# mitschabaude/msm-zprize

Measured on AMD Instinct MI355X. Metric: Mpoint-adds/s (ms per MSM in ms_per_step), higher is better.
Workload: dtype u32 limbs (28-bit lazy Montgomery, i64 accumulate)

## Files before the change

### msm_zprize_amd/_native.py

```python
import ctypes as C
import os

HERE = os.path.dirname(os.path.abspath(__file__))
LIB_PATH = os.environ.get("MSMZ_LIB") or os.path.join(HERE, "libmsmz.so")

MSMZ_N_STAGES = 8
STAGE_NAMES = ["digits", "scan", "scatter", "plan", "accumulate", "reduce", "final", "total"]


class MsmzOpts(C.Structure):
    _fields_ = [("c", C.c_int32), ("glv", C.c_int32), ("safe", C.c_int32), ("buckets", C.c_int32),
                ("timing", C.c_int32), ("reserved", C.c_int32 * 3)]


class MsmzLog(C.Structure):
    _fields_ = [("stage_ms", C.c_float * MSMZ_N_STAGES), ("c", C.c_int32), ("K", C.c_int32), ("rounds", C.c_int32),
                ("glv", C.c_int32), ("n_entries", C.c_uint64), ("n_pairs", C.c_uint64), ("max_bucket", C.c_uint32),
                ("scatter_launches", C.c_uint32), ("scatter_kernel_ms", C.c_float), ("batch_add_ms", C.c_float * 32)]


MSMZ_SRC_DEVICE, MSMZ_SRC_MONTGOMERY, MSMZ_SRC_DEFAULT_STREAM = 1, 2, 4
MSMZ_SRC_COMPRESSED, MSMZ_SRC_SIGN_PARITY = 8, 16
MSMZ_ERR_POINT = 7

# ... 24 lines not shown


class MsmzScalarTerm(C.Structure):
    _fields_ = [("handle", C.c_uint64), ("first", C.c_uint64), ("coeff_handle", C.c_uint64), ("coeff_first", C.c_uint64),
                ("coeff", C.c_char_p)]


MSMZ_REC_REVERSE, MSMZ_REC_EXCLUSIVE = 1, 2


class MsmzScalarRec(C.Structure):
    _fields_ = [("a_handle", C.c_uint64), ("a_first", C.c_uint64), ("a", C.c_char_p), ("b_handle", C.c_uint64),
                ("b_first", C.c_uint64), ("init", C.c_char_p), ("flags", C.c_uint32)]


MSMZ_NTT_INVERSE, MSMZ_NTT_COSET = 1, 2


class MsmzNtt(C.Structure):
    _fields_ = [("handle", C.c_uint64), ("first", C.c_uint64), ("log_n", C.c_uint32), ("flags", C.c_uint32),
                ("n_in", C.c_uint64), ("count", C.c_uint32), ("root", C.c_char_p), ("shift", C.c_char_p)]


class MsmzSegment(C.Structure):
    _fields_ = [("first_p", C.c_uint64), ("first_s", C.c_uint64), ("n", C.c_uint64)]


class MsmzTestReduceArgs(C.Structure):
    _fields_ = [("mode", C.c_int32), ("c", C.c_int32), ("nsets", C.c_uint32), ("n_in", C.c_uint32),
                ("nc", C.c_uint32), ("tail_n", C.c_uint32), ("quad16_max", C.c_uint32), ("pairsum_x4_max", C.c_uint32),
                ("points_xy", C.c_char_p), ("points_inf", C.c_char_p), ("n_points", C.c_uint64),
                ("slots_xy", C.c_char_p), ("slots_inf", C.c_char_p), ("n_slots", C.c_uint64),
                ("scale", C.c_char_p), ("loc", C.c_void_p), ("cscan", C.c_void_p),
                ("out_xy", C.c_void_p), ("lines_xy", C.c_void_p)]


class MsmzTestPlanArgs(C.Structure):
    _fields_ = [("nb", C.c_uint32), ("chunk", C.c_uint32), ("nb_main", C.c_uint32), ("chunk_top", C.c_uint32),
                ("tail_skip", C.c_int32), ("reserved", C.c_uint32),
                ("off", C.c_void_p), ("refs", C.c_void_p),
                ("desc_cap", C.c_uint64), ("bfin_cap", C.c_uint64), ("chunk_pairs_cap", C.c_uint64),
                ("meta", C.c_void_p), ("desc", C.c_void_p), ("bfin", C.c_void_p), ("chunk_pairs", C.c_void_p)]


class MsmzTestSortArgs(C.Structure):
    _fields_ = [("scalars_le32", C.c_void_p), ("n", C.c_uint64), ("pts_n", C.c_uint64),
                ("nprob", C.c_uint32), ("factor", C.c_uint32), ("copy_stride", C.c_uint32),
                ("c", C.c_int32), ("glv", C.c_int32), ("force_fallback", C.c_int32), ("scalar_bits", C.c_int32),
                ("allow_fold", C.c_int32),
                ("geom_cap", C.c_uint64), ("off_cap", C.c_uint64), ("refs_cap", C.c_uint64), ("bins_cap", C.c_uint64),
                ("packed_cap", C.c_uint64),
                ("geom", C.c_void_p), ("meta", C.c_void_p), ("off", C.c_void_p), ("refs", C.c_void_p),
                ("bins", C.c_void_p), ("packed", C.c_void_p)]


TEST_SORT_GEOM = ["c", "K", "Keff", "L", "nb", "fb", "fbt", "ncb", "ncbt", "nbins", "sbins", "fbins", "fine_top", "spread",
                  "fold_shift", "fold_rows", "F", "mbits", "idx_bits", "cspec", "two_level", "tiles", "sbits", "endo_delta"]


EXPORTS = {
    "msmz_create": (C.c_int, [C.POINTER(C.c_void_p), C.c_int, C.POINTER(C.c_int), C.c_int]),
    "msmz_destroy": (None, [C.c_void_p]),
    "msmz_strerror": (C.c_char_p, [C.c_int]),
    "msmz_curve_fe_bytes": (C.c_int, [C.c_int]),
    "msmz_ctx_fe_bytes": (C.c_int, [C.c_void_p]),
    "msmz_ctx_n_devices": (C.c_int, [C.c_void_p]),
    "msmz_upload_points": (C.c_int, [C.c_void_p, C.c_char_p, C.c_char_p, C.c_uint64, C.POINTER(C.c_uint64)]),
# ... 21 lines not shown
                                    C.POINTER(MsmzOpts), C.c_char_p, C.POINTER(C.c_int), C.POINTER(MsmzLog)]),
    "msmz_precompute_points": (C.c_int, [C.c_void_p, C.c_uint64, C.c_uint64, C.POINTER(MsmzOpts), C.c_uint32,
                                         C.POINTER(C.c_uint64)]),
    "msmz_precomputed_info": (C.c_int, [C.c_void_p, C.c_uint64, C.POINTER(C.c_int32), C.POINTER(C.c_int32),
                                        C.POINTER(C.c_uint32), C.POINTER(C.c_uint32), C.POINTER(C.c_uint64)]),
    "msmz_precomputed_scalar_bits": (C.c_int, [C.c_void_p, C.c_uint64, C.POINTER(C.c_int32)]),
    "msmz_check_points": (C.c_int, [C.c_void_p, C.c_uint64, C.c_uint64, C.c_uint64, C.c_uint32,
                                    C.POINTER(MsmzCheckResult), C.c_char_p]),
    "msmz_points_mul": (C.c_int, [C.c_void_p, C.POINTER(MsmzMul), C.c_uint64, C.POINTER(C.c_uint64)]),
    "msmz_points_mul_opts": (C.c_int, [C.c_void_p, C.POINTER(MsmzMul), C.c_uint64, C.POINTER(MsmzMulOpts),
                                       C.POINTER(C.c_uint64)]),
    "msmz_scalars_combine": (C.c_int, [C.c_void_p, C.POINTER(MsmzScalarTerm), C.POINTER(MsmzScalarTerm), C.c_uint64,
                                       C.c_uint64, C.POINTER(C.c_uint64)]),
    "msmz_scalars_dot": (C.c_int, [C.c_void_p, C.c_uint64, C.c_uint64, C.c_uint64, C.c_uint64, C.c_uint64, C.c_char_p]),
    "msmz_scalars_powers": (C.c_int, [C.c_void_p, C.c_char_p, C.c_char_p, C.c_uint64, C.POINTER(C.c_uint64)]),
    "msmz_scalars_recurrence": (C.c_int, [C.c_void_p, C.POINTER(MsmzScalarRec), C.c_uint64, C.c_uint64,
                                          C.POINTER(C.c_uint64), C.c_char_p]),
    "msmz_scalars_inverse": (C.c_int, [C.c_void_p, C.c_uint64, C.c_uint64, C.c_uint64, C.c_uint64, C.POINTER(C.c_uint64),
                                       C.POINTER(C.c_uint64)]),
    "msmz_scalars_ntt": (C.c_int, [C.c_void_p, C.POINTER(MsmzNtt), C.c_uint64, C.POINTER(C.c_uint64)]),
    "msmz_scalars_root_of_unity": (C.c_int, [C.c_int, C.c_uint32, C.c_char_p]),
    "msmz_point_add": (C.c_int, [C.c_int, C.c_char_p, C.c_int, C.c_char_p, C.c_int, C.c_char_p, C.POINTER(C.c_int)]),
    "msmz_test_set_glv_bits": (C.c_int, [C.c_void_p, C.c_int]),
    "msmz_test_retries": (C.c_int, [C.c_void_p]),
    "msmz_test_set_limits": (C.c_int, [C.c_void_p, C.c_uint64, C.c_uint64]),
    "msmz_test_passes": (C.c_int, [C.c_void_p, C.POINTER(C.c_uint64), C.POINTER(C.c_uint64)]),
    "msmz_test_scalar_dot_geometry": (None, [C.POINTER(C.c_uint32), C.POINTER(C.c_uint32)]),
    "msmz_test_scalar_scan_geometry": (None, [C.POINTER(C.c_uint32), C.POINTER(C.c_uint32), C.POINTER(C.c_uint32)]),
    "msmz_test_ntt_plan": (C.c_int, [C.c_int, C.c_uint32, C.POINTER(C.c_uint32), C.POINTER(C.c_uint32)]),
    "msmz_test_ntt_geometry": (None, [C.POINTER(C.c_uint32)]),
    "msmz_test_field": (C.c_int, [C.c_void_p, C.c_int, C.c_char_p, C.c_char_p, C.c_uint64, C.c_char_p]),
    "msmz_test_field_limbs": (C.c_int, [C.c_void_p, C.c_int, C.c_void_p, C.c_void_p, C.c_uint64, C.c_void_p,
                                        C.c_char_p]),
    "msmz_test_glv": (C.c_int, [C.c_void_p, C.c_char_p, C.c_uint64, C.c_char_p, C.c_char_p, C.c_char_p]),
    "msmz_test_digits": (C.c_int, [C.c_void_p, C.c_char_p, C.c_uint64, C.c_int, C.c_int, C.c_int, C.c_void_p]),
    "msmz_test_sort": (C.c_int, [C.c_void_p, C.c_char_p, C.c_uint64, C.c_int, C.c_int, C.c_int, C.c_void_p, C.c_void_p,
                                 C.c_uint64, C.c_void_p, C.c_uint64]),
    "msmz_test_sort_ex": (C.c_int, [C.c_void_p, C.POINTER(MsmzTestSortArgs)]),
    "msmz_test_point_raw": (C.c_int, [C.c_void_p, C.c_int, C.c_char_p, C.c_char_p, C.c_char_p, C.c_uint64, C.c_int,
                                      C.c_char_p]),
    "msmz_test_point": (C.c_int, [C.c_void_p, C.c_int, C.c_char_p, C.c_char_p, C.c_char_p, C.c_char_p, C.c_uint64,
                                  C.c_char_p]),
    "msmz_test_batch_add": (C.c_int, [C.c_void_p, C.c_int, C.c_int, C.c_char_p, C.c_char_p, C.c_uint64, C.c_char_p,
                                      C.c_char_p, C.c_uint64, C.c_void_p, C.c_uint64, C.c_uint64, C.c_char_p,
                                      C.POINTER(C.c_uint32)]),
    "msmz_test_reduce": (C.c_int, [C.c_void_p, C.POINTER(MsmzTestReduceArgs)]),
    "msmz_test_plan": (C.c_int, [C.c_void_p, C.POINTER(MsmzTestPlanArgs)]),
}

_lib = None


class MsmzError(RuntimeError):
    def __init__(self, status, where):
        self.status = status
        msg = lib().msmz_strerror(status).decode() if _lib is not None else "?"
        super().__init__(f"{where}: msmz status {status} ({msg})")


def lib():
    global _lib
    if _lib is None:
        if not os.path.exists(LIB_PATH):
            raise RuntimeError(f"{LIB_PATH} is missing: run `python -m msm_zprize_amd.build` "
                               "(the MSM has no CPU fallback)")
        l = C.CDLL(LIB_PATH)
# ... 12 lines not shown
```

### msm_zprize_amd/csrc/instantiate.h

```cpp
#pragma once
#include "check_kernels.h"
#include "gen_kernels.h"
#include "import_kernels.h"
#include "kernels.h"
#include "mul_kernels.h"
#include "ntt_kernels.h"
#include "scalar_kernels.h"
#include "scan_kernels.h"
#include "test_kernels.h"

#if !defined(MSMZ_CURVE) || MSMZ_CURVE == 0
#define MSMZ_W0(X) X(Bls377Fp, Bls377Fr)
#else
#define MSMZ_W0(X)
#endif
#if !defined(MSMZ_CURVE) || MSMZ_CURVE == 1
#define MSMZ_W1(X) X(PallasFp, PallasFr)
#else
#define MSMZ_W1(X)
#endif
#if !defined(MSMZ_CURVE) || MSMZ_CURVE == 2
#define MSMZ_W2(X) X(Bls381Fp, Bls381Fr)
#else
#define MSMZ_W2(X)
#endif
#if !defined(MSMZ_CURVE) || MSMZ_CURVE == 3
#define MSMZ_T3(X) X(Ed377Fp, Ed377Fr)
#else
#define MSMZ_T3(X)
#endif
#define MSMZ_WEIERSTRASS_FIELDS(X) MSMZ_W0(X) MSMZ_W1(X) MSMZ_W2(X)
#define MSMZ_TE_FIELDS(X) MSMZ_T3(X)

#ifndef MSMZ_BATCH_T
#define MSMZ_BATCH_T 256
#endif
#ifndef MSMZ_BATCH_OCC
#define MSMZ_BATCH_OCC 4
#endif
#ifndef MSMZ_BATCH_BMAX
#define MSMZ_BATCH_BMAX 16
#endif

#define MSMZ_INST_BATCH(F, Fr, PFX)                                                                               \
  PFX template __global__ void k_batch_add<F, MSMZ_BATCH_T, true, MSMZ_BATCH_OCC, MSMZ_BATCH_BMAX>(              \
      uint32_t*, const uint32_t*, const uint2*, uint32_t, uint32_t, int, MsmMeta*);                              \
  PFX template __global__ void k_batch_add<F, MSMZ_BATCH_T, false, MSMZ_BATCH_OCC, MSMZ_BATCH_BMAX>(             \
      uint32_t*, const uint32_t*, const uint2*, uint32_t, uint32_t, int, MsmMeta*);

#define MSMZ_INST_POLICY(P, PFX)                                                                                 \
  PFX template __global__ void k_reduce_quad<P>(uint32_t*, uint32_t*, const uint32_t*, const uint32_t*, uint32_t, \
                                                uint32_t, uint32_t);                                             \
  PFX template __global__ void k_reduce_quad16<P>(uint32_t*, uint32_t*, const uint32_t*, const uint32_t*,        \
                                                  uint32_t, uint32_t, uint32_t);                                 \
  PFX template __global__ void k_reduce_tail<P>(uint32_t*, uint32_t*, uint32_t*, uint32_t*, uint32_t*, uint32_t, \
                                                uint32_t);                                                       \
  PFX template __global__ void k_pairsum<P>(uint32_t*, const uint32_t*, uint32_t);                               \
  PFX template __global__ void k_fill_neutral<P>(uint32_t*, uint32_t);                                           \
  PFX template __global__ void k_bucket_sums<P>(uint32_t*, const uint32_t*, const uint32_t*, uint32_t);          \
  PFX template __global__ void k_reduce2d_partial_acc<P>(uint32_t*, const uint32_t*, const uint32_t*, R2Geom, uint32_t); \
  PFX template __global__ void k_pairsum_x4<P>(uint32_t*, const uint32_t*, uint32_t);                            \
  PFX template __global__ void k_bucket_accumulate<P>(uint32_t*, const uint32_t*, const uint32_t*,               \
                                                      const uint32_t*, const uint32_t*, uint32_t, uint32_t, int);

#define MSMZ_INST_REDUCE(F, Fr, PFX)                                                                              \
  PFX template __global__ void k_reduce2d_partial<F>(uint32_t*, const uint32_t*, const uint32_t*, const uint4*,   \
                                                     R2Geom, uint32_t);                                          \
  PFX template __global__ void k_reduce_affine_finish<F>(uint32_t*, uint32_t*, const uint32_t*, const uint32_t*,  \
                                                         const uint2*, const uint4*, F2Geom);                     \
  MSMZ_INST_POLICY(WeierPolicy<F>, PFX)

#define MSMZ_INST_REDUCE_TE(F, Fr, PFX) MSMZ_INST_POLICY(TePolicy<F>, PFX)

#define MSMZ_INST_TEST(F, Fr, P, PFX)                                                                             \
  PFX template __global__ void k_test_field<F>(uint32_t*, const uint32_t*, const uint32_t*, uint32_t, int, uint32_t*); \
  PFX template __global__ void k_test_field_limbs<F>(int32_t*, uint32_t*, const int32_t*, const int32_t*, uint32_t,  \
                                                      int, uint32_t*);                                            \
  PFX template __global__ void k_test_glv<Fr>(uint32_t*, uint32_t*, uint8_t*, const uint32_t*, uint32_t);         \
  PFX template __global__ void k_test_digits<Fr, false>(uint32_t*, const uint32_t*, uint32_t, int, int);          \
  PFX template __global__ void k_test_point<P>(uint32_t*, const uint32_t*, const uint32_t*, const uint8_t*,   \
                                                   const uint8_t*, uint32_t, int);                                \
  PFX template __global__ void k_test_point_raw<P>(uint32_t*, const uint32_t*, const uint32_t*, const uint8_t*, \
                                                       uint32_t, int, int);                                       \
  PFX template __global__ void k_test_accs_in<P>(uint32_t*, const uint32_t*, const uint8_t*, const uint32_t*, \
                                                     uint32_t, uint32_t*);                                        \
  PFX template __global__ void k_test_accs_out<P>(uint32_t*, const uint32_t*, uint32_t);

#define MSMZ_INST_SORT(Fr, PFX, GLV, C, SEG)                                                                      \
  PFX template __global__ void k_hist<Fr, GLV, C, SEG>(uint32_t*, uint16_t*, uint32_t*, MsmMeta*, const uint32_t*, SortGeom, uint32_t, const SegDesc*); \
  PFX template __global__ void k_coarse<Fr, GLV, C, SEG>(uint32_t*, const uint32_t*, const uint32_t*, const uint16_t*, const uint32_t*, SortGeom, uint32_t, const SegDesc*);

#define MSMZ_INST_SCAN(Fr, AM, HB, PFX)                                                                           \
  PFX template __global__ void k_scalars_rec_tile<Fr, AM, HB>(uint32_t*, uint32_t*, const uint32_t*, const uint32_t*, FrConst, uint32_t, uint32_t, uint32_t*); \
  PFX template __global__ void k_scalars_rec_apply<Fr, AM, HB>(uint32_t*, const uint32_t*, const uint32_t*, FrConst, const uint32_t*, uint32_t, uint32_t);

#define MSMZ_INST_SCALAR(Fr, PFX)                                                                                 \
  PFX template __global__ void k_digits<Fr, false>(uint32_t*, uint32_t*, MsmMeta*, const uint32_t*, uint32_t, int, int, int, int); \
  MSMZ_SORT_INSTANCES(MSMZ_INST_SORT, Fr, PFX)                                                                    \
  PFX template __global__ void k_check_scalars<Fr>(uint32_t*, const uint32_t*, uint32_t);                         \
  PFX template __global__ void k_gen_scalars<Fr>(uint32_t*, uint32_t, uint64_t, GenMap);                          \
  PFX template __global__ void k_import_scalars<Fr>(uint32_t*, const uint8_t*, uint64_t, int, uint32_t, int, uint32_t*); \
  PFX template __global__ void k_scalars_combine<Fr>(uint32_t*, ScalarTerm, ScalarTerm, uint32_t, uint32_t*);     \
  PFX template __global__ void k_scalars_dot<Fr>(uint32_t*, const uint32_t*, const uint32_t*, uint32_t, uint32_t*); \
  PFX template __global__ void k_scalars_dot_fold<Fr>(uint32_t*, const uint32_t*, uint32_t, int);                 \
  PFX template __global__ void k_scalars_powers<Fr>(uint32_t*, FrConst, FrPowTable, uint32_t, GenMap);                \
  MSMZ_INST_SCAN(Fr, SREC_A_NONE, true, PFX)                                                                      \
  MSMZ_INST_SCAN(Fr, SREC_A_BROADCAST, false, PFX)                                                                \
  MSMZ_INST_SCAN(Fr, SREC_A_BROADCAST, true, PFX)                                                                 \
  MSMZ_INST_SCAN(Fr, SREC_A_RESIDENT, false, PFX)                                                                 \
  MSMZ_INST_SCAN(Fr, SREC_A_RESIDENT, true, PFX)                                                                  \
// ... 40 lines not shown
```

### msm_zprize_amd/csrc/kernels.h

```cpp
#pragma once
#include <hip/hip_runtime.h>
#include "constants_gen.h"
#include "plan.h"
#include "curve.h"
#include "scalar.h"

namespace msmz {

constexpr uint32_t REF_NEG = 0x80000000u;
constexpr uint32_t REF_IDX = 0x7fffffffu;

struct MsmMeta {
  uint32_t max_bucket;
  uint32_t n_entries;
  uint32_t error;
  uint32_t rounds;
  uint32_t round_pairs[32];
  uint32_t round_base[32];
};

typedef uint32_t u32x4 __attribute__((ext_vector_type(4)));

#ifndef MSMZ_POINT_PAD
#define MSMZ_POINT_PAD 1
#endif
template <class F>
struct PointFmt {
  static constexpr int STRIDE = (MSMZ_POINT_PAD && 2 * F::NW == 24) ? 32 : 2 * F::NW;
};

constexpr bool SLOT_NT = false;
template <class F, bool NT = false>
__device__ __forceinline__ void load_words(uint32_t* dst, const uint32_t* src, int cs = 1) {
  const u32x4* s4 = reinterpret_cast<const u32x4*>(src);
#pragma unroll
  for (int i = 0; i < (2 * F::NW) / 4; i++) {
    u32x4 v = NT ? __builtin_nontemporal_load(s4 + i * cs) : s4[i * cs];
// ... 367 lines not shown
template <class F>
__device__ __forceinline__ void load_operand_x(Fe<F>& x, uint32_t loc, const uint32_t* slots, const uint32_t* points) {
  if constexpr (SlotFmt<F>::PACKED) {
    int cs;
    uint32_t neg;
    const u32x4* s4 = reinterpret_cast<const u32x4*>(operand_address<F>(loc, slots, points, cs, neg));
    uint32_t w[F::NW];
#pragma unroll
    for (int i = 0; i < F::NW / 4; i++) {
      const u32x4 v = s4[i * cs];
      w[4 * i] = v.x;
      w[4 * i + 1] = v.y;
      w[4 * i + 2] = v.z;
      w[4 * i + 3] = v.w;
    }
    fe_unpack<F>(x, w);
  } else {
    if (loc & LOC_ORIG) {
      uint32_t w[F::NW];
      const u32x4* s4 = reinterpret_cast<const u32x4*>(points + (size_t)(loc & 0x3fffffffu) * PointFmt<F>::STRIDE);
#pragma unroll
      for (int i = 0; i < F::NW / 4; i++) {
        const u32x4 v = s4[i];
        w[4 * i] = v.x;
        w[4 * i + 1] = v.y;
        w[4 * i + 2] = v.z;
        w[4 * i + 3] = v.w;
      }
      fe_unpack<F>(x, w);
    } else {
      slot_load_fe<F>(x, slots + slot_offset<F>(loc));
    }
  }
}

template <int W, int N>
__device__ __forceinline__ int32_t limb_row_ripple(int32_t val, int j) {
  constexpr int32_t MASK = (1 << W) - 1;
  const bool low = j < N - 1;
#pragma unroll 1
  for (int pass = 0; pass < N - 1; pass++) {
    const int32_t c = low ? (val >> W) : 0;
    val = low ? (val & MASK) : val;
    val += __builtin_amdgcn_update_dpp(0, c, 0x111, 0xf, 0xf, true);
    if (__ballot(low && (uint32_t)val > (uint32_t)MASK) == 0) break;
  }
  return val;
}

template <class F>
__device__ __forceinline__ bool fe_inverse_wave(Fe<F>& r, const Fe<F>& x) {
  constexpr int N = F::N, W = F::W;
  constexpr uint32_t MASK = (1u << W) - 1u;
  static_assert(N <= 15, "one DPP row per vector");
  const int lane = (int)(threadIdx.x & 63u);
  const int row = lane >> 4, j = lane & 15;
  int32_t xl = 0, pl = 0, npl = 0;
  {
    Fe<F> xc;
    uint32_t w[F::NW];
    fe_to_canon_words<F>(w, x);
    fe_unpack<F>(xc, w);
#pragma unroll
    for (int k = 0; k < N; k++) {
      if (j == k) {
        xl = xc.l[k];
        pl = F::PL[k];
        npl = F::NPL[k];
      }
    }
  }
  int32_t val = row == 0 ? xl : row == 1 ? pl : (row == 2 && j == 0) ? 1 : 0;
  constexpr int ITERS = (2 * F::BITS + W - 1) / W + 1;
#pragma unroll 1
  for (int it = 0; it < ITERS; it++) {
    const uint64_t nz = __ballot(val != 0);
    const uint32_t ma = (uint32_t)nz & 0xffffu, mb = (uint32_t)(nz >> 16) & 0xffffu;
    if (ma == 0) break;
    const int h = 31 - __builtin_clz(ma | mb | 1u);
    const uint32_t a0 = (uint32_t)__builtin_amdgcn_readlane(val, 0), b0 = (uint32_t)__builtin_amdgcn_readlane(val, 16);
// ... 181 lines not shown
  fe_carry(t);
  fe_carry(u);
  fe_add(v, p.Y, p.X);
  fe_add(w, q.Y, q.X);
  fe_carry(v);
  fe_carry(w);
  fe_sel4(a, s, t, v, p.T, p.Z);
  fe_sel4(b, s, u, w, q.T, q.Z);
  fe_mul(m, a, b);
  fe_quad_bcast<0>(A, m);
  fe_quad_bcast<1>(B, m);
  fe_quad_bcast<2>(t, m);
  fe_quad_bcast<3>(D, m);
  fe_set_const<F>(k, F::K2D);
  fe_mul(C, t, k);
  fe_add(D, D, D);
  fe_sub(E, B, A);
  fe_sub(Fv, D, C);
  fe_add(G, D, C);
  fe_add(H, B, A);
  fe_carry(E);
  fe_carry(Fv);
  fe_carry(G);
  fe_carry(H);
  fe_sel4(a, s, E, G, E, Fv);
  fe_sel4(b, s, Fv, H, H, G);
  fe_mul(m, a, b);
  fe_quad_bcast<0>(r.X, m);
  fe_quad_bcast<1>(r.Y, m);
  fe_quad_bcast<2>(r.T, m);
  fe_quad_bcast<3>(r.Z, m);
}

template <class F_>
struct WeierPolicy : WeierGroup<F_> {
  using G = WeierGroup<F_>;
  using F = F_;
  using typename G::Acc;
  using typename G::Base;
  using G::madd;
  static constexpr int IN_WORDS = PointFmt<F>::STRIDE;
  static constexpr int ACC_WORDS = 4 * F::NW;
  static constexpr int ACC_OCC = 1;
  static __device__ __forceinline__ void add_x4(Acc& r, const Acc& a, const Acc& b, int s, bool dbl) { xyzz_add_x4(r, a, b, s, dbl); }
  static __device__ __forceinline__ void madd(Acc& r, const Acc& a, const uint32_t* rec, uint32_t neg) {
    Affine<F> p;
    bool inf = load_affine<F>(p, rec, neg);
    xyzz_madd(r, a, p, inf);
  }
  static __device__ __forceinline__ void load(Acc& a, const uint32_t* rec) { load_fe4<F>(a.X, a.Y, a.ZZ, a.ZZZ, rec); }
  static __device__ __forceinline__ void store(uint32_t* rec, const Acc& a) { store_fe4<F>(rec, a.X, a.Y, a.ZZ, a.ZZZ); }
  static __device__ __forceinline__ bool load_base(Base& b, const uint32_t* rec) {
    return b.inf = load_affine<F>(b.a, rec, 0);
  }
  static __device__ __forceinline__ bool load_resident_affine(Fe<F>& x, Fe<F>& y, const uint32_t* rec) {
    Affine<F> a;
    const bool inf = load_affine<F>(a, rec, 0);
    x = a.x;
    y = a.y;
    return inf;
  }
  static __device__ __forceinline__ void store_resident(uint32_t* out, uint32_t i, uint32_t n, const Fe<F>& x,
                                                        const Fe<F>& y, bool flagged, int endo) {
    Affine<F> m{x, y};
    store_affine<F>(out + (size_t)i * IN_WORDS, m, flagged);
    if (endo) {
      if (!flagged) {
        Fe<F> beta;
        fe_set_const<F>(beta, F::BETA);
        fe_mul(m.x, x, beta);
      }
      store_affine<F>(out + ((size_t)n + i) * IN_WORDS, m, flagged);
    }
  }
  static __device__ __forceinline__ void store_normalised(uint32_t* out, uint32_t i, uint32_t n, const Acc& a,
                                                          const Fe<F>& zi3, bool dead, int endo) {
    Fe<F> x, y;
    fe_zero(x);
    fe_zero(y);
    if (!dead) G::affine_from_inverse(x, y, a, zi3);
    store_resident(out, i, n, x, y, dead, endo);
  }
};

template <class F_>
struct TePolicy : TeGroup<F_> {
  using G = TeGroup<F_>;
  using F = F_;
  using typename G::Acc;
  using typename G::Base;
  using G::madd;
  static constexpr int IN_WORDS = 4 * F::NW;
  static constexpr int ACC_WORDS = 4 * F::NW;
  static constexpr int ACC_OCC = 1;
  static __device__ __forceinline__ void add_x4(Acc& r, const Acc& a, const Acc& b, int s, bool dbl) { te_add_x4(r, a, b, s, dbl); }
  static __device__ __forceinline__ void madd(Acc& r, const Acc& a, const uint32_t* rec, uint32_t neg) {
    Base n;
    Fe<F> x;
    load_fe4<F>(n.ym, n.yp, n.kt, x, rec);
    te_madd(r, a, n, neg);
  }
  static __device__ __forceinline__ void load(Acc& a, const uint32_t* rec) { load_fe4<F>(a.X, a.Y, a.Z, a.T, rec); }
  static __device__ __forceinline__ void store(uint32_t* rec, const Acc& a) { store_fe4<F>(rec, a.X, a.Y, a.Z, a.T); }
  static __device__ __forceinline__ bool load_base(Base& b, const uint32_t* rec) {
    Fe<F> x;
    load_fe4<F>(b.ym, b.yp, b.kt, x, rec);
    return false;
  }
  static __device__ __forceinline__ bool load_resident_affine(Fe<F>& x, Fe<F>& y, const uint32_t* rec) {
    Base b;
    load_fe4<F>(b.ym, b.yp, b.kt, x, rec);
    fe_add(y, b.ym, x);
    return false;
  }
  static __device__ __forceinline__ void store_resident(uint32_t* out, uint32_t i, uint32_t , const Fe<F>& x,
                                                        const Fe<F>& y, bool , int ) {
    Base b;
    G::base_from_affine(b, x, y, false);
    store_fe4<F>(out + (size_t)i * IN_WORDS, b.ym, b.yp, b.kt, x);
  }
  static __device__ __forceinline__ void store_normalised(uint32_t* out, uint32_t i, uint32_t n, const Acc& a,
                                                          const Fe<F>& zi, bool dead, int endo) {
    Fe<F> x, y;
    if (dead) {
      fe_zero(x);
      fe_set_const<F>(y, F::ONE);
    } else {
      G::affine_from_inverse(x, y, a, zi);
// ... 202 lines not shown
  reduce_group16<P>(rows_out + (size_t)k * groups * XW, c_out + (size_t)k * groups * XW,
                    rows_in + (size_t)k * n_in * XW, c_in + (size_t)k * n_in * XW, n_in, A, live, q, s, base_lane);
}

constexpr int REDUCE_TAIL_T = 256;
constexpr uint32_t REDUCE_TAIL_N = 32;
template <class P>
__global__ void __launch_bounds__(REDUCE_TAIL_T, 1) k_reduce_tail(uint32_t* r0, uint32_t* c0, uint32_t* r1, uint32_t* c1,
                                                                  uint32_t* c_final, uint32_t n_in, uint32_t stride) {
  constexpr int XW = P::ACC_WORDS;
  const uint32_t k = blockIdx.x;
  uint32_t* rin = r0 + (size_t)k * stride * XW;
  uint32_t* cin = c0 + (size_t)k * stride * XW;
  uint32_t* rout = r1 + (size_t)k * stride * XW;
  uint32_t* cout = c1 + (size_t)k * stride * XW;
  const uint32_t q = (threadIdx.x >> 2) & 3;
  const int s = (int)(threadIdx.x & 3);
  const int lane = threadIdx.x & 63, base_lane = (lane & ~15) + s;
  uint32_t n = n_in;
  while (n > 1) {
    const uint32_t g2 = (n + 3) / 4;
    for (uint32_t A0 = 0; A0 < g2; A0 += REDUCE_TAIL_T / 16) {
      const uint32_t A = A0 + (threadIdx.x >> 4);
      reduce_group16<P>(rout, cout, rin, cin, n, A, A < g2, q, s, base_lane);
    }
    __syncthreads();
    uint32_t* t1 = rin; rin = rout; rout = t1;
    uint32_t* t2 = cin; cin = cout; cout = t2;
    n = g2;
  }
  for (uint32_t j = threadIdx.x; j < (uint32_t)XW; j += REDUCE_TAIL_T) c_final[(size_t)k * XW + j] = cin[j];
}


}

#include "reduce_affine.h"
#include "reduce2d_kernels.h"
```

### msm_zprize_amd/csrc/msmz.hip

```cpp
#include "instantiate.h"
namespace msmz {
#define X(F, Fr) MSMZ_INST_BATCH(F, Fr, MSMZ_EXTERN) MSMZ_INST_REDUCE(F, Fr, MSMZ_EXTERN) MSMZ_INST_MISC(F, Fr, MSMZ_EXTERN) MSMZ_INST_GEN(F, Fr, MSMZ_EXTERN)
MSMZ_WEIERSTRASS_FIELDS(X)
#undef X
#define X(F, Fr) MSMZ_INST_REDUCE_TE(F, Fr, MSMZ_EXTERN) MSMZ_INST_MISC_TE(F, Fr, MSMZ_EXTERN) MSMZ_INST_GEN_TE(F, Fr, MSMZ_EXTERN)
MSMZ_TE_FIELDS(X)
#undef X
}
#include "test_hooks.h"

namespace msmz {

template <class F_, class Fr_>
struct WeierCfg {
  using F = F_;
  using Fr = Fr_;
  using P = WeierPolicy<F>;
  static constexpr bool TE = false;
  static constexpr bool HAS_ENDO = true;
};

template <class F_, class Fr_>
struct TeCfg {
  using F = F_;
// ... 252 lines not shown
  for (uint32_t j = 0; j < 8; j++) stages[j] = j < p.n_passes ? p.pass[j].s : 0;
  return MSMZ_OK;
}
void msmz_test_ntt_geometry(uint32_t* pass_log) {
  if (pass_log) *pass_log = NTT_PASS_LOG;
}
void msmz_test_scalar_dot_geometry(uint32_t* tile_elements, uint32_t* partials_per_pass) {
  if (tile_elements) *tile_elements = SDOT_TILE;
  if (partials_per_pass) *partials_per_pass = SDOT_PASS;
}
void msmz_test_scalar_scan_geometry(uint32_t* rec_tile, uint32_t* rec_pass, uint32_t* inv_chunk) {
  if (rec_tile) *rec_tile = SREC_TILE;
  if (rec_pass) *rec_pass = SREC_PASS;
  if (inv_chunk) *inv_chunk = SINV_CHUNK;
}

int msmz_test_set_glv_bits(msmz_ctx* c, int bits) { return c ? c->engine->test_set_glv_bits(bits) : MSMZ_ERR_ARG; }
int msmz_test_retries(msmz_ctx* c) { return c ? c->engine->test_retries() : -1; }
int msmz_test_set_limits(msmz_ctx* c, uint64_t pass_entries, uint64_t batch_entries) {
  return c ? c->engine->test_set_limits(pass_entries, batch_entries) : MSMZ_ERR_ARG;
}
int msmz_test_passes(msmz_ctx* c, uint64_t* range_passes, uint64_t* sub_batches) {
  if (!c) return MSMZ_ERR_ARG;
  c->engine->test_passes(range_passes, sub_batches);
  return MSMZ_OK;
}
int msmz_test_field(msmz_ctx* c, int op, const uint8_t* a, const uint8_t* b, uint64_t n, uint8_t* out) {
  return c ? c->engine->test_hooks()->test_field(op, a, b, n, out) : MSMZ_ERR_ARG;
}
int msmz_test_field_limbs(msmz_ctx* c, int op, const int32_t* a, const int32_t* b, uint64_t n, int32_t* raw,
                          uint8_t* canon) {
  return c ? c->engine->test_hooks()->test_field_limbs(op, a, b, n, raw, canon) : MSMZ_ERR_ARG;
}
int msmz_test_glv(msmz_ctx* c, const uint8_t* s, uint64_t n, uint8_t* s0, uint8_t* s1, uint8_t* neg) {
  return c ? c->engine->test_hooks()->test_glv(s, n, s0, s1, neg) : MSMZ_ERR_ARG;
}
int msmz_test_digits(msmz_ctx* c, const uint8_t* s, uint64_t n, int cc, int K, int glv, uint32_t* digits) {
  return c ? c->engine->test_hooks()->test_digits(s, n, cc, K, glv, digits) : MSMZ_ERR_ARG;
}
int msmz_test_sort(msmz_ctx* c, const uint8_t* s, uint64_t n, int cc, int glv, int force_fallback, uint32_t* geom,
                   uint32_t* off, uint64_t off_cap, uint32_t* refs, uint64_t refs_cap) {
  if (!c) return MSMZ_ERR_ARG;
  return c->engine->test_hooks()->test_sort(s, n, cc, glv, force_fallback, geom, off, off_cap, refs, refs_cap);
}
int msmz_test_sort_ex(msmz_ctx* c, const msmz_test_sort_args* a) {
  return c && a ? c->engine->test_hooks()->test_sort_ex(*a) : MSMZ_ERR_ARG;
}
int msmz_test_point_raw(msmz_ctx* c, int op, const uint8_t* a, const uint8_t* b, const uint8_t* neg, uint64_t n, int L,
                        uint8_t* out) {
  return c ? c->engine->test_hooks()->test_point_raw(op, a, b, neg, n, L, out) : MSMZ_ERR_ARG;
}
int msmz_test_point(msmz_ctx* c, int op, const uint8_t* a, const uint8_t* ai, const uint8_t* b, const uint8_t* bi,
                    uint64_t n, uint8_t* out) {
  return c ? c->engine->test_hooks()->test_point(op, a, ai, b, bi, n, out) : MSMZ_ERR_ARG;
}

int msmz_test_batch_add(msmz_ctx* c, int safe, int B, const uint8_t* pxy, const uint8_t* pinf, uint64_t np,
                        const uint8_t* sxy, const uint8_t* sinf, uint64_t ns, const uint32_t* desc, uint64_t n_pairs,
                        uint64_t out_base, uint8_t* out, uint32_t* error) {
  if (!c) return MSMZ_ERR_ARG;
  return c->engine->test_hooks()->test_batch_add(safe, B, pxy, pinf, np, sxy, sinf, ns, desc, n_pairs, out_base, out, error);
}

int msmz_test_reduce(msmz_ctx* c, const msmz_test_reduce_args* a) {
  return c && a ? c->engine->test_hooks()->test_reduce(*a) : MSMZ_ERR_ARG;
}
// ... 18 lines not shown
```

### msm_zprize_amd/csrc/reduce.h

```cpp
#pragma once
#include <hip/hip_runtime.h>

#include <cstring>

#include "../../include/msmz.h"
#include "batch_add.h"
#include "kernels.h"
#include "plan.h"
#include "store.h"

namespace msmz {

struct ReduceKnobs {
  uint32_t tail_n = (uint32_t)env_int("MSMZ_TAIL_N", REDUCE_TAIL_N);
  uint32_t quad16_max = (uint32_t)env_int("MSMZ_QUAD16", 8192);
  uint32_t pairsum_x4_max = (uint32_t)env_int("MSMZ_PAIRSUM_X4", 16384);
};

struct BucketSource {
  const uint32_t* recs;
  const uint32_t* points;
  const uint4* bfin;
  const uint32_t* cscan;

  static BucketSource locations(const uint32_t* slots, const uint32_t* pts, const uint4* bfin) { return {slots, pts, bfin, nullptr}; }
  static BucketSource chunks(const uint32_t* accs, const uint32_t* cscan) { return {accs, nullptr, nullptr, cscan}; }
  static BucketSource per_bucket(const uint32_t* accs) { return {accs, nullptr, nullptr, nullptr}; }
};

template <class Cfg>
class BucketReduce {
  using F = typename Cfg::F;
  using P = typename Cfg::P;
  static constexpr int AW = P::ACC_WORDS;

 public:
  int run_2d(const R2Geom& g, const ReduceKnobs& rk, const BucketSource& src, hipStream_t stream) {
    const uint32_t* lines;
    if (int st = line_sums(g, rk, src, stream, &lines)) return st;
    return weighted_sums(g, rk, stream);
  }

  int line_sums(const R2Geom& g, const ReduceKnobs& rk, const BucketSource& src, hipStream_t stream,
                const uint32_t** lines) {
    const uint32_t n_lines = g.nprob * g.H;
    const uint32_t total = n_lines * g.NC;
    int st;
    if ((st = rows_room(0, total)) || (st = rows_room(1, total))) return st;
    if (src.bfin) {
// ... 8 lines not shown
    for (uint32_t n = total / 2; n >= n_lines && g.NC > 1; n /= 2) {
      if (n <= rk.pairsum_x4_max) {
        hipLaunchKernelGGL((k_pairsum_x4<P>), dim3((n * 4 + 63) / 64), dim3(64), 0, stream, rows(cur_ ^ 1), rows(cur_), n);
      } else {
        hipLaunchKernelGGL((k_pairsum<P>), dim3((n + 127) / 128), dim3(128), 0, stream, rows(cur_ ^ 1), rows(cur_), n);
      }
      cur_ ^= 1;
      if (n == n_lines) break;
    }
    *lines = rows(cur_);
    return MSMZ_OK;
  }

  int weighted_sums(const R2Geom& g, const ReduceKnobs& rk, hipStream_t stream) {
    const uint32_t n_lines = g.nprob * g.H;
    if (int st = carry_room(cur_, n_lines)) return st;
    hipLaunchKernelGGL((k_fill_neutral<P>), dim3((n_lines + 255) / 256), dim3(256), 0, stream, carry(cur_), n_lines);
    if (int st = levels(rk, g.H, g.nprob, stream)) return st;
    MSMZ_HIP(hipGetLastError());
    return MSMZ_OK;
  }

  int level_inputs(size_t n, uint32_t** rows_out, uint32_t** c_out) {
    int st;
    if ((st = rows_room(0, n)) || (st = carry_room(0, n))) return st;
    cur_ = 0;
    *rows_out = rows(0);
    *c_out = carry(0);
    return MSMZ_OK;
  }

  int levels(const ReduceKnobs& rk, uint32_t n_in, uint32_t nprob, hipStream_t stream) {
    int st;
    while (n_in > rk.tail_n) {
      const uint32_t S = 4;
      const uint32_t g2 = (n_in + S - 1) / S;
      const int nxt = cur_ ^ 1;
      if ((st = rows_room(nxt, (size_t)nprob * g2)) || (st = carry_room(nxt, (size_t)nprob * g2))) return st;
      const uint32_t total = nprob * g2;
      if (total <= rk.quad16_max) {
        hipLaunchKernelGGL((k_reduce_quad16<P>), dim3((total * 16 + 63) / 64), dim3(64), 0, stream, rows(nxt), carry(nxt),
                           rows(cur_), carry(cur_), n_in, g2, total);
      } else {
        hipLaunchKernelGGL((k_reduce_quad<P>), dim3((total * 4 + 63) / 64), dim3(64), 0, stream, rows(nxt), carry(nxt),
                           rows(cur_), carry(cur_), n_in, g2, total);
      }
      n_in = g2;
      cur_ = nxt;
    }
    const int nxt = cur_ ^ 1;
    if ((st = rows_room(nxt, (size_t)nprob * n_in)) || (st = carry_room(nxt, (size_t)nprob * n_in))) return st;
    if ((st = final_.ensure((size_t)nprob * AW * 4))) return st;
    hipLaunchKernelGGL((k_reduce_tail<P>), dim3(nprob), dim3(REDUCE_TAIL_T), 0, stream, rows(cur_), carry(cur_), rows(nxt),
                       carry(nxt), final_.as<uint32_t>(), n_in, n_in);
    return MSMZ_OK;
  }

  int bucket_sums(BucketSource chunks, uint32_t nb, hipStream_t stream, BucketSource* sums) {
    if (int st = bsum_.ensure((size_t)nb * AW * 4)) return st;
    hipLaunchKernelGGL((k_bucket_sums<P>), dim3((nb + 127) / 128), dim3(128), 0, stream, bsum_.as<uint32_t>(), chunks.recs,
                       chunks.cscan, nb);
    *sums = BucketSource::per_bucket(bsum_.as<uint32_t>());
    return MSMZ_OK;
  }

  int first_affine(const Plan& pl, uint32_t S, uint32_t groups, uint64_t tree_pairs, const BatchAdder<Cfg>& adder,
                   size_t slot_bytes, const BucketSource& src, MsmMeta* d_meta) {
    F2Geom g;
    memset(&g, 0, sizeof(g));
    g.L = pl.L;
    g.S = S;
    g.groups = groups;
    g.NG = (uint32_t)pl.Keff * groups;
// ... 47 lines not shown
```

Before: 4641.

## Add DPP row-parallel field arithmetic and row-based small-level reduce kernel

```diff
diff --git a/msm_zprize_amd/_native.py b/msm_zprize_amd/_native.py
--- a/msm_zprize_amd/_native.py
+++ b/msm_zprize_amd/_native.py
@@ -80,7 +80,7 @@
                 ("points_xy", C.c_char_p), ("points_inf", C.c_char_p), ("n_points", C.c_uint64),
                 ("slots_xy", C.c_char_p), ("slots_inf", C.c_char_p), ("n_slots", C.c_uint64),
                 ("scale", C.c_char_p), ("loc", C.c_void_p), ("cscan", C.c_void_p),
-                ("out_xy", C.c_void_p), ("lines_xy", C.c_void_p)]
+                ("out_xy", C.c_void_p), ("lines_xy", C.c_void_p), ("rows_max", C.c_uint32)]
 
 
 class MsmzTestPlanArgs(C.Structure):
@@ -168,6 +168,8 @@
     "msmz_test_field": (C.c_int, [C.c_void_p, C.c_int, C.c_char_p, C.c_char_p, C.c_uint64, C.c_char_p]),
     "msmz_test_field_limbs": (C.c_int, [C.c_void_p, C.c_int, C.c_void_p, C.c_void_p, C.c_uint64, C.c_void_p,
                                         C.c_char_p]),
+    "msmz_test_field_rows": (C.c_int, [C.c_void_p, C.c_int, C.c_void_p, C.c_void_p, C.c_uint64, C.c_uint32, C.c_void_p,
+                                       C.c_char_p]),
     "msmz_test_glv": (C.c_int, [C.c_void_p, C.c_char_p, C.c_uint64, C.c_char_p, C.c_char_p, C.c_char_p]),
     "msmz_test_digits": (C.c_int, [C.c_void_p, C.c_char_p, C.c_uint64, C.c_int, C.c_int, C.c_int, C.c_void_p]),
     "msmz_test_sort": (C.c_int, [C.c_void_p, C.c_char_p, C.c_uint64, C.c_int, C.c_int, C.c_int, C.c_void_p, C.c_void_p,
diff --git a/msm_zprize_amd/csrc/fp_rows.h b/msm_zprize_amd/csrc/fp_rows.h
--- /dev/null
+++ b/msm_zprize_amd/csrc/fp_rows.h
@@ -0,0 +1,178 @@
+#pragma once
+#include "fp.h"
+
+#if defined(__HIPCC__)
+namespace msmz {
+
+template <class F>
+struct RowLane {
+  int j;
+  int32_t pl;
+  int32_t npl;
+  int32_t p2;
+  int32_t one;
+};
+
+template <class F>
+__device__ __forceinline__ int32_t row_const(const int32_t (&c)[F::N], int j) {
+  int32_t v = 0;
+#pragma unroll
+  for (int i = 0; i < F::N; i++) v = j == i ? c[i] : v;
+  return v;
+}
+
+template <class F>
+__device__ __forceinline__ RowLane<F> row_lane() {
+  static_assert(F::N <= 15, "one DPP row per element");
+  RowLane<F> k;
+  k.j = (int)(__lane_id() & 15u);
+  k.pl = row_const<F>(F::PL, k.j);
+  k.npl = -k.pl;
+  k.p2 = row_const<F>(F::P2, k.j);
+  k.one = row_const<F>(F::ONE, k.j);
+  return k;
+}
+
+template <int I>
+__device__ __forceinline__ int32_t row_bcast(int32_t x) {
+  return __builtin_amdgcn_update_dpp(0, x, 0x150 + I, 0xf, 0xf, false);
+}
+__device__ __forceinline__ int32_t row_down1(int32_t x) {
+  return __builtin_amdgcn_update_dpp(0, x, 0x101, 0xf, 0xf, true);
+}
+__device__ __forceinline__ int32_t row_up1(int32_t x) {
+  return __builtin_amdgcn_update_dpp(0, x, 0x111, 0xf, 0xf, true);
+}
+
+template <int W, int N>
+__device__ __forceinline__ int32_t limb_row_ripple(int32_t val, int j) {
+  constexpr int32_t MASK = (1 << W) - 1;
+  const bool low = j < N - 1;
+#pragma unroll 1
+  for (int pass = 0; pass < N - 1; pass++) {
+    const int32_t c = low ? (val >> W) : 0;
+    val = low ? (val & MASK) : val;
+    val += row_up1(c);
+    if (__ballot(low && (uint32_t)val > (uint32_t)MASK) == 0) break;
+  }
+  return val;
+}
+
+
+template <class F>
+__device__ __forceinline__ int32_t fe_carry_row(int32_t a, const RowLane<F>& k) {
+  constexpr int32_t MASK = (1 << F::W) - 1;
+  const bool low = k.j < F::N - 1;
+  const int32_t c = low ? (a >> F::W) : 0;
+  return (low ? (a & MASK) : a) + row_up1(c);
+}
+
+__device__ __forceinline__ int32_t fe_select_row(bool c, int32_t a, int32_t b) { return c ? a : b; }
+
+template <class F, int I>
+struct RowMulStep {
+  static __device__ __forceinline__ void run(int64_t& acc, int32_t a, int32_t b, int32_t npl) {
+    constexpr uint32_t MASK = (1u << F::W) - 1u;
+    int32_t ai = row_bcast<I>(a);
+    MSMZ_OPAQUE_LIMB(ai);
+    acc += (int64_t)ai * (int64_t)b;
+    uint32_t q = (uint32_t)row_bcast<0>((int32_t)(uint32_t)acc);
+    if (F::PINV != 1u) q *= F::PINV;
+    int32_t m = (int32_t)(q & MASK);
+    MSMZ_OPAQUE_LIMB(m);
+    acc += (int64_t)m * (int64_t)npl;
+    const int32_t lo = (int32_t)((uint32_t)acc & MASK);
+    acc = (acc >> F::W) + (int64_t)row_down1(lo);
+    if constexpr (I + 1 < F::N) RowMulStep<F, I + 1>::run(acc, a, b, npl);
+  }
+};
+
+template <class F>
+__device__ __forceinline__ int32_t fe_mul_row(int32_t a, int32_t b, const RowLane<F>& k) {
+  constexpr int N = F::N, W = F::W;
+  constexpr uint32_t MASK = (1u << W) - 1u;
+  int32_t npl = k.npl;
+  MSMZ_OPAQUE_LIMB(b);
+  MSMZ_OPAQUE_LIMB(npl);
+  int64_t acc = 0;
+  RowMulStep<F, 0>::run(acc, a, b, npl);
+  const bool low = k.j < N - 1;
+  const int32_t c = low ? (int32_t)(acc >> W) : 0;
+  int32_t v = low ? (int32_t)((uint32_t)acc & MASK) : (int32_t)acc;
+  v += row_up1(c);
+  return limb_row_ripple<W, N>(v, k.j);
+}
+
+template <class F>
+__device__ __forceinline__ int32_t fe_sqr_row(int32_t a, const RowLane<F>& k) {
+  return fe_mul_row<F>(a, a, k);
+}
+
+template <class F>
+__device__ __forceinline__ int32_t fe_reduce_small_row(int32_t a, const RowLane<F>& k) {
+  constexpr int N = F::N, W = F::W;
+  constexpr uint32_t MASK = (1u << W) - 1u;
+  const int32_t est = row_bcast<N - 1>(a) + (row_bcast<N - 2>(a) >> W);
+  constexpr int SH = (F::PL[N - 1] >= (1 << 16)) ? 8 : 0;
+  const float x = (float)(est >> SH) * (1.0f / (float)((F::PL[N - 1] >> SH) + 1));
+  const int32_t q = (int32_t)__builtin_floorf(x) - 1;
+  const int64_t t = (int64_t)a + (int64_t)q * (int64_t)k.npl;
+  const bool low = k.j < N - 1;
+  const int32_t c = low ? (int32_t)(t >> W) : 0;
+  int32_t v = low ? (int32_t)((uint32_t)t & MASK) : (int32_t)t;
+  v += row_up1(c);
+  return limb_row_ripple<W, N>(v, k.j);
+}
+
+template <class F>
+__device__ __forceinline__ bool fe_is_zero_row(int32_t a, const RowLane<F>& k) {
+  if constexpr (F::PL[0] == 1) {
+    constexpr uint32_t MASK = (1u << F::W) - 1u;
+    if (__ballot(k.j == 0 && (((uint32_t)a + 15u) & MASK) <= 30u) == 0) return false;
+  }
+  const int32_t v = fe_reduce_small_row<F>(a, k);
+  const int sh = (int)(__lane_id() & 48u);
+  const uint32_t n0 = (uint32_t)(__ballot(v != 0) >> sh) & 0xffffu;
+  const uint32_t n1 = (uint32_t)(__ballot(v != k.pl) >> sh) & 0xffffu;
+  const uint32_t n2 = (uint32_t)(__ballot(v != k.p2) >> sh) & 0xffffu;
+  return n0 == 0 || n1 == 0 || n2 == 0;
+}
+
+template <class F>
+__device__ __forceinline__ int32_t fe_load_row(const uint32_t* w, const RowLane<F>& k) {
+  constexpr int N = F::N, W = F::W, NW = F::NW;
+  constexpr uint32_t MASK = (1u << W) - 1u;
+  if (k.j >= N) return 0;
+  const int bit = W * k.j;
+  const int w0 = bit >> 5, sh = bit & 31;
+  uint32_t v = w[w0] >> sh;
+  if (sh + W > 32 && w0 + 1 < NW) v |= w[w0 + 1] << (32 - sh);
+  return (int32_t)(v & MASK);
+}
+
+template <class F>
+__device__ __forceinline__ void fe_pack_row(uint32_t* w, int32_t a, const RowLane<F>& k, bool write = true) {
+  constexpr int W = F::W, NW = F::NW;
+  static_assert((32 * (NW - 1)) / W + 2 <= 15, "a word's limbs lie within the row");
+  const int i = k.j < NW ? k.j : 0;
+  const int j0 = (32 * i) / W, o = 32 * i - W * j0;
+  const int base = (int)(__lane_id() & 48u) + j0;
+  const uint32_t l0 = (uint32_t)__shfl(a, base, 64);
+  const uint32_t l1 = (uint32_t)__shfl(a, base + 1, 64);
+  const uint32_t l2 = (uint32_t)__shfl(a, base + 2, 64);
+  uint32_t v = (l0 >> o) | (l1 << (W - o));
+  if (2 * W - o < 32) v |= l2 << (2 * W - o);
+  if (write && k.j < NW) w[k.j] = v;
+}
+
+template <class F>
+__device__ __forceinline__ void fe_store_row(uint32_t* w, int32_t a, const RowLane<F>& k, bool write = true) {
+  fe_pack_row<F>(w, fe_reduce_small_row<F>(a, k), k, write);
+}
+
+__device__ __forceinline__ int32_t fe_from_row(int32_t a, int src_row) {
+  return __shfl(a, src_row * 16 + (int)(__lane_id() & 15u), 64);
+}
+
+}
+#endif
diff --git a/msm_zprize_amd/csrc/instantiate.h b/msm_zprize_amd/csrc/instantiate.h
--- a/msm_zprize_amd/csrc/instantiate.h
+++ b/msm_zprize_amd/csrc/instantiate.h
@@ -55,6 +55,8 @@
                                                   uint32_t, uint32_t, uint32_t);                                 \
   PFX template __global__ void k_reduce_tail<P>(uint32_t*, uint32_t*, uint32_t*, uint32_t*, uint32_t*, uint32_t, \
                                                 uint32_t);                                                       \
+  PFX template __global__ void k_reduce_rows<P>(uint32_t*, uint32_t*, const uint32_t*, const uint32_t*, uint32_t, \
+                                                uint32_t, uint32_t);                                             \
   PFX template __global__ void k_pairsum<P>(uint32_t*, const uint32_t*, uint32_t);                               \
   PFX template __global__ void k_fill_neutral<P>(uint32_t*, uint32_t);                                           \
   PFX template __global__ void k_bucket_sums<P>(uint32_t*, const uint32_t*, const uint32_t*, uint32_t);          \
@@ -76,6 +78,8 @@
   PFX template __global__ void k_test_field<F>(uint32_t*, const uint32_t*, const uint32_t*, uint32_t, int, uint32_t*); \
   PFX template __global__ void k_test_field_limbs<F>(int32_t*, uint32_t*, const int32_t*, const int32_t*, uint32_t,  \
                                                       int, uint32_t*);                                            \
+  PFX template __global__ void k_test_field_rows<F>(int32_t*, uint32_t*, const int32_t*, const int32_t*, uint32_t,   \
+                                                     int, uint32_t);                                              \
   PFX template __global__ void k_test_glv<Fr>(uint32_t*, uint32_t*, uint8_t*, const uint32_t*, uint32_t);         \
   PFX template __global__ void k_test_digits<Fr, false>(uint32_t*, const uint32_t*, uint32_t, int, int);          \
   PFX template __global__ void k_test_point<P>(uint32_t*, const uint32_t*, const uint32_t*, const uint8_t*,   \
diff --git a/msm_zprize_amd/csrc/kernels.h b/msm_zprize_amd/csrc/kernels.h
--- a/msm_zprize_amd/csrc/kernels.h
+++ b/msm_zprize_amd/csrc/kernels.h
@@ -3,6 +3,7 @@
 #include "constants_gen.h"
 #include "plan.h"
 #include "curve.h"
+#include "fp_rows.h"
 #include "scalar.h"
 
 namespace msmz {
@@ -436,20 +437,6 @@
       slot_load_fe<F>(x, slots + slot_offset<F>(loc));
     }
   }
-}
-
-template <int W, int N>
-__device__ __forceinline__ int32_t limb_row_ripple(int32_t val, int j) {
-  constexpr int32_t MASK = (1 << W) - 1;
-  const bool low = j < N - 1;
-#pragma unroll 1
-  for (int pass = 0; pass < N - 1; pass++) {
-    const int32_t c = low ? (val >> W) : 0;
-    val = low ? (val & MASK) : val;
-    val += __builtin_amdgcn_update_dpp(0, c, 0x111, 0xf, 0xf, true);
-    if (__ballot(low && (uint32_t)val > (uint32_t)MASK) == 0) break;
-  }
-  return val;
 }
 
 template <class F>
@@ -697,6 +684,110 @@
   fe_quad_bcast<3>(r.Z, m);
 }
 
+template <class F>
+struct AccRow {
+  int32_t c[4];
+};
+
+__device__ __forceinline__ int32_t row_sel4(int s, int32_t a0, int32_t a1, int32_t a2, int32_t a3) {
+  const int32_t lo = (s & 1) ? a1 : a0, hi = (s & 1) ? a3 : a2;
+  return (s & 2) ? hi : lo;
+}
+
+template <class F>
+__device__ __forceinline__ void acc_load_row(AccRow<F>& a, const uint32_t* rec, const RowLane<F>& k) {
+#pragma unroll
+  for (int i = 0; i < 4; i++) a.c[i] = fe_load_row<F>(rec + i * F::NW, k);
+}
+
+template <class F>
+__device__ __forceinline__ void acc_store_row(uint32_t* rec, const AccRow<F>& a, const RowLane<F>& k) {
+  const bool write = (__lane_id() & 48u) == 0;
+#pragma unroll
+  for (int i = 0; i < 4; i++) fe_store_row<F>(rec + i * F::NW, a.c[i], k, write);
+}
+
+template <class F>
+__device__ __forceinline__ void xyzz_core_rows(AccRow<F>& r, const AccRow<F>& p, const AccRow<F>& q, bool dbl,
+                                               int32_t& P, int32_t& R, const RowLane<F>& k) {
+  const int s = (int)(__lane_id() >> 4);
+  const int32_t pX = p.c[0], pY = p.c[1], pZZ = p.c[2], pZZZ = p.c[3];
+  const int32_t qX = q.c[0], qY = q.c[1], qZZ = q.c[2], qZZZ = q.c[3];
+  int32_t m = fe_mul_row<F>(row_sel4(s, pX, qX, pY, qY), row_sel4(s, qZZ, pZZ, qZZZ, pZZZ), k);
+  const int32_t U1 = fe_from_row(m, 0), U2 = fe_from_row(m, 1), S1 = fe_from_row(m, 2), S2 = fe_from_row(m, 3);
+  P = U2 - U1;
+  R = S2 - S1;
+  const int32_t U = fe_carry_row<F>(pY + pY, k);
+  int32_t a = row_sel4(s, P, R, pZZ, pZZZ), b = row_sel4(s, P, R, qZZ, qZZZ);
+  int32_t t = (s & 1) ? pX : U;
+  m = fe_mul_row<F>(dbl ? t : a, dbl ? t : b, k);
+  const int32_t PP = fe_from_row(m, 0);
+  int32_t RR = fe_from_row(m, 1);
+  const int32_t Zm = fe_from_row(m, 2), Zc = fe_from_row(m, 3);
+  const int32_t M = fe_carry_row<F>(RR + RR + RR, k);
+  a = row_sel4(s, P, U1, Zm, Zm);
+  t = row_sel4(s, U, pX, M, pZZ);
+  m = fe_mul_row<F>(dbl ? t : a, (dbl && s == 2) ? M : PP, k);
+  const int32_t PPP = fe_from_row(m, 0);
+  const int32_t Q = fe_from_row(m, 1);
+  t = fe_from_row(m, 2);
+  int32_t u = fe_from_row(m, 3);
+  r.c[2] = dbl ? u : t;
+  RR = dbl ? t : RR;
+  u = fe_carry_row<F>(RR - (dbl ? 0 : PPP) - Q - Q, k);
+  t = fe_carry_row<F>(Q - u, k);
+  a = row_sel4(s, R, S1, Zc, Zc);
+  m = row_sel4(s, M, pY, pZZZ, pZZZ);
+  m = fe_mul_row<F>(dbl ? m : a, s == 0 ? t : PPP, k);
+  r.c[3] = fe_from_row(m, 2);
+  r.c[1] = fe_carry_row<F>(fe_from_row(m, 0) - fe_from_row(m, 1), k);
+  r.c[0] = u;
+}
+
+template <class F>
+__device__ __forceinline__ void xyzz_add_rows(AccRow<F>& r, const AccRow<F>& p, const AccRow<F>& q, bool dbl,
+                                              const RowLane<F>& k) {
+  const bool pinf = fe_is_zero_row<F>(p.c[2], k), qinf = fe_is_zero_row<F>(q.c[2], k);
+  int32_t P, R;
+  xyzz_core_rows<F>(r, p, q, dbl, P, R, k);
+  if (pinf) {
+    r = q;
+  } else if (qinf) {
+    r = p;
+  } else if (!dbl && fe_is_zero_row<F>(P, k)) {
+    if (fe_is_zero_row<F>(R, k)) {
+      xyzz_core_rows<F>(r, p, p, true, P, R, k);
+    } else {
+      r.c[0] = k.one;
+      r.c[1] = k.one;
+      r.c[2] = 0;
+      r.c[3] = 0;
+    }
+  }
+}
+
+template <class F>
+__device__ __forceinline__ void te_add_rows(AccRow<F>& r, const AccRow<F>& p, const AccRow<F>& q, bool,
+                                            const RowLane<F>& k) {
+  const int s = (int)(__lane_id() >> 4);
+  const int32_t pX = p.c[0], pY = p.c[1], pZ = p.c[2], pT = p.c[3];
+  const int32_t qX = q.c[0], qY = q.c[1], qZ = q.c[2], qT = q.c[3];
+  const int32_t t = fe_carry_row<F>(pY - pX, k), u = fe_carry_row<F>(qY - qX, k);
+  const int32_t v = fe_carry_row<F>(pY + pX, k), w = fe_carry_row<F>(qY + qX, k);
+  int32_t m = fe_mul_row<F>(row_sel4(s, t, v, pT, pZ), row_sel4(s, u, w, qT, qZ), k);
+  const int32_t A = fe_from_row(m, 0), B = fe_from_row(m, 1), TT = fe_from_row(m, 2);
+  int32_t D = fe_from_row(m, 3);
+  const int32_t C = fe_mul_row<F>(TT, row_const<F>(F::K2D, k.j), k);
+  D = D + D;
+  const int32_t E = fe_carry_row<F>(B - A, k), Fv = fe_carry_row<F>(D - C, k);
+  const int32_t G = fe_carry_row<F>(D + C, k), H = fe_carry_row<F>(B + A, k);
+  m = fe_mul_row<F>(row_sel4(s, E, G, E, Fv), row_sel4(s, Fv, H, H, G), k);
+  r.c[0] = fe_from_row(m, 0);
+  r.c[1] = fe_from_row(m, 1);
+  r.c[3] = fe_from_row(m, 2);
+  r.c[2] = fe_from_row(m, 3);
+}
+
 template <class F_>
 struct WeierPolicy : WeierGroup<F_> {
   using G = WeierGroup<F_>;
@@ -708,6 +799,9 @@
   static constexpr int ACC_WORDS = 4 * F::NW;
   static constexpr int ACC_OCC = 1;
   static __device__ __forceinline__ void add_x4(Acc& r, const Acc& a, const Acc& b, int s, bool dbl) { xyzz_add_x4(r, a, b, s, dbl); }
+  using Row = AccRow<F>;
+  static __device__ __forceinline__ void add_rows(Row& r, const Row& a, const Row& b, bool dbl, const RowLane<F>& k) { xyzz_add_rows(r, a, b, dbl, k); }
+  static __device__ __forceinline__ void identity_row(Row& a, const RowLane<F>& k) { a.c[0] = a.c[1] = k.one; a.c[2] = a.c[3] = 0; }
   static __device__ __forceinline__ void madd(Acc& r, const Acc& a, const uint32_t* rec, uint32_t neg) {
     Affine<F> p;
     bool inf = load_affine<F>(p, rec, neg);
@@ -759,6 +853,9 @@
   static constexpr int ACC_WORDS = 4 * F::NW;
   static constexpr int ACC_OCC = 1;
   static __device__ __forceinline__ void add_x4(Acc& r, const Acc& a, const Acc& b, int s, bool dbl) { te_add_x4(r, a, b, s, dbl); }
+  using Row = AccRow<F>;
+  static __device__ __forceinline__ void add_rows(Row& r, const Row& a, const Row& b, bool dbl, const RowLane<F>& k) { te_add_rows(r, a, b, dbl, k); }
+  static __device__ __forceinline__ void identity_row(Row& a, const RowLane<F>& k) { a.c[0] = a.c[3] = 0; a.c[1] = a.c[2] = k.one; }
   static __device__ __forceinline__ void madd(Acc& r, const Acc& a, const uint32_t* rec, uint32_t neg) {
     Base n;
     Fe<F> x;
@@ -1027,6 +1124,74 @@
   for (uint32_t j = threadIdx.x; j < (uint32_t)XW; j += REDUCE_TAIL_T) c_final[(size_t)k * XW + j] = cin[j];
 }
 
+constexpr int ROWS_PUB_WORDS = 2 * 4 * 4 * 16;
+template <class P>
+__device__ __forceinline__ void reduce_group_rows(uint32_t* rows_out, uint32_t* c_out, const uint32_t* rows_in,
+                                                  const uint32_t* c_in, uint32_t n_in, uint32_t A, bool live, uint32_t q,
+                                                  int32_t* pub, const RowLane<typename P::F>& rk) {
+  using F = typename P::F;
+  using Row = typename P::Row;
+  constexpr int XW = P::ACC_WORDS;
+  const uint32_t e = A * 4 + q;
+  const int lj = (int)(__lane_id() & 15u);
+  Row r, c, v, w, got, ident;
+  P::identity_row(ident, rk);
+  r = ident;
+  c = ident;
+  if (live && e < n_in) {
+    acc_load_row<F>(r, rows_in + (size_t)e * XW, rk);
+    acc_load_row<F>(c, c_in + (size_t)e * XW, rk);
+  }
+  auto exchange = [&](int step, const Row& mine, uint32_t src) {
+    int32_t* buf = pub + (step & 1) * (4 * 4 * 16);
+    if (__lane_id() < 16u) {
+#pragma unroll
+      for (int i = 0; i < 4; i++) buf[(q * 4 + i) * 16 + lj] = mine.c[i];
+    }
+    __syncthreads();
+#pragma unroll
+    for (int i = 0; i < 4; i++) got.c[i] = buf[(src * 4 + i) * 16 + lj];
+  };
+  {
+    const uint32_t src[4] = {1, 3, 3, 2};
+    exchange(0, q == 2 ? c : r, src[q]);
+    P::add_rows(v, q == 3 ? c : r, got, false, rk);
+  }
+  {
+    const uint32_t src[4] = {2, 0, 2, 3};
+    exchange(1, q == 0 ? c : v, src[q]);
+    if (q == 3) got = ident;
+    Row lhs = (q == 1) ? c : v;
+    if (q == 3) lhs = ident;
+    P::add_rows(w, lhs, got, q == 2, rk);
+  }
+  {
+    const uint32_t src[4] = {0, 3, 1, 3};
+    exchange(2, q == 0 ? w : v, src[q]);
+    P::add_rows(r, w, got, q == 0, rk);
+  }
+  {
+    const uint32_t src[4] = {0, 2, 2, 3};
+    exchange(3, r, src[q]);
+    P::add_rows(c, r, got, q == 0, rk);
+  }
+  if (live && q == 0) acc_store_row<F>(rows_out + (size_t)A * XW, c, rk);
+  if (live && q == 1) acc_store_row<F>(c_out + (size_t)A * XW, c, rk);
+}
+
+template <class P>
+__global__ void __launch_bounds__(256) k_reduce_rows(uint32_t* rows_out, uint32_t* c_out, const uint32_t* rows_in,
+                                                     const uint32_t* c_in, uint32_t n_in, uint32_t groups, uint32_t total) {
+  constexpr int XW = P::ACC_WORDS;
+  __shared__ int32_t pub[ROWS_PUB_WORDS];
+  const RowLane<typename P::F> rk = row_lane<typename P::F>();
+  const uint32_t grp = blockIdx.x;
+  const uint32_t k = grp / groups, A = grp - k * groups;
+  reduce_group_rows<P>(rows_out + (size_t)k * groups * XW, c_out + (size_t)k * groups * XW,
+                       rows_in + (size_t)k * n_in * XW, c_in + (size_t)k * n_in * XW, n_in, A, true, threadIdx.x >> 6,
+                       pub, rk);
+}
+
 
 }
 
diff --git a/msm_zprize_amd/csrc/msmz.hip b/msm_zprize_amd/csrc/msmz.hip
--- a/msm_zprize_amd/csrc/msmz.hip
+++ b/msm_zprize_amd/csrc/msmz.hip
@@ -308,6 +308,10 @@
                           uint8_t* canon) {
   return c ? c->engine->test_hooks()->test_field_limbs(op, a, b, n, raw, canon) : MSMZ_ERR_ARG;
 }
+int msmz_test_field_rows(msmz_ctx* c, int op, const int32_t* a, const int32_t* b, uint64_t n, uint32_t live_rows,
+                         int32_t* raw, uint8_t* canon) {
+  return c ? c->engine->test_hooks()->test_field_rows(op, a, b, n, live_rows, raw, canon) : MSMZ_ERR_ARG;
+}
 int msmz_test_glv(msmz_ctx* c, const uint8_t* s, uint64_t n, uint8_t* s0, uint8_t* s1, uint8_t* neg) {
   return c ? c->engine->test_hooks()->test_glv(s, n, s0, s1, neg) : MSMZ_ERR_ARG;
 }
diff --git a/msm_zprize_amd/csrc/reduce.h b/msm_zprize_amd/csrc/reduce.h
--- a/msm_zprize_amd/csrc/reduce.h
+++ b/msm_zprize_amd/csrc/reduce.h
@@ -15,6 +15,7 @@
   uint32_t tail_n = (uint32_t)env_int("MSMZ_TAIL_N", REDUCE_TAIL_N);
   uint32_t quad16_max = (uint32_t)env_int("MSMZ_QUAD16", 8192);
   uint32_t pairsum_x4_max = (uint32_t)env_int("MSMZ_PAIRSUM_X4", 16384);
+  uint32_t rows_max = (uint32_t)env_int("MSMZ_ROWS_MAX", 512);
 };
 
 struct BucketSource {
@@ -89,13 +90,17 @@
 
   int levels(const ReduceKnobs& rk, uint32_t n_in, uint32_t nprob, hipStream_t stream) {
     int st;
-    while (n_in > rk.tail_n) {
+    const uint32_t rows_max = rk.rows_max < rk.quad16_max ? rk.rows_max : rk.quad16_max;
+    while (n_in > rk.tail_n || (n_in > 1 && (uint64_t)nprob * ((n_in + 3) / 4) <= rows_max)) {
       const uint32_t S = 4;
       const uint32_t g2 = (n_in + S - 1) / S;
       const int nxt = cur_ ^ 1;
       if ((st = rows_room(nxt, (size_t)nprob * g2)) || (st = carry_room(nxt, (size_t)nprob * g2))) return st;
       const uint32_t total = nprob * g2;
-      if (total <= rk.quad16_max) {
+      if (total <= rows_max) {
+        hipLaunchKernelGGL((k_reduce_rows<P>), dim3(total), dim3(256), 0, stream, rows(nxt), carry(nxt), rows(cur_),
+                           carry(cur_), n_in, g2, total);
+      } else if (total <= rk.quad16_max) {
         hipLaunchKernelGGL((k_reduce_quad16<P>), dim3((total * 16 + 63) / 64), dim3(64), 0, stream, rows(nxt), carry(nxt),
                            rows(cur_), carry(cur_), n_in, g2, total);
       } else {
```

After: 4823 (median of 6 runs). 1.04x the previous value.
